# bminixhofer/zett

Measured on AMD Instinct MI355X. Metric: predicted token-embeddings/sec (full target vocab), higher is better.
Workload: dtype f16

## Files before the change

zett_amd/csrc/rowops.hip.h:

```cpp
#pragma once

#include <hip/hip_runtime.h>
#include <stdint.h>

#include <type_traits>

#include "gemm.hip.h"
#include "scan.hip.h"

namespace zett {



struct PlanArrays {
    int32_t* row_count;
    int32_t* row_offset;
    uint8_t* row_uniform;
    int32_t* id_flag;
    int32_t* id_slot;
    int32_t* id_list;
    int32_t* tok_slot;
    int32_t* tok_pos;
    int32_t* tok_row;
    int32_t* tok_pkey;
    int32_t* pair_flag;
    int32_t* pair_slot;
    int32_t* tok_pair;
    int32_t* pair_tslot;
    int32_t* pair_pos;
    uint8_t* tok_key;
    int32_t* err;
    int32_t* counters;
    int32_t n_pair_keys;
};

static __global__ void plan_rows_kernel(const int32_t* __restrict__ sfm, int64_t n_rows, int seq, int pad, int lam,
                                 int n_ids, PlanArrays p) {
    const int64_t n = (int64_t)blockIdx.x * blockDim.x + threadIdx.x;
    if (n >= n_rows) return;
    const int32_t* row = sfm + n * seq;
    int visible = 0;
    for (int j = 0; j < seq; ++j) {
        const int id = row[j];
        if (id < 0 || id >= n_ids) {
            atomicMax(p.err, (int)(n < 0x7ffffffe ? n + 1 : 0x7fffffff));
            p.row_count[n] = 0;
            p.row_uniform[n] = 2;
            return;
        }
        visible += (id != pad);
    }
    const bool uniform = (visible + lam) == 0;
    int count;
    if (uniform) {
        count = seq;
        for (int j = 0; j < seq; ++j) p.id_flag[row[j]] = 1;
    } else {
        count = visible + lam + (row[0] == pad ? 1 : 0);
        for (int j = 0; j < seq; ++j)
            if (j == 0 || row[j] != pad) p.id_flag[row[j]] = 1;
    }
    p.row_count[n] = count;
    p.row_uniform[n] = uniform ? 1 : 0;
}

static __global__ __launch_bounds__(1024) void exclusive_scan_kernel(const int32_t* __restrict__ in,
                                                              int32_t* __restrict__ out, int64_t n) {
    __shared__ int32_t s_waves[16];
    const int t = threadIdx.x;
    const int64_t per = (n + 1023) / 1024;
    const int64_t b = (int64_t)t * per, e = (b + per < n) ? b + per : n;
    int32_t s = 0;
    for (int64_t i = b; i < e; ++i) s += in[i];
    int32_t total;
    int32_t run = block_exclusive_scan<1024>(s, s_waves, &total);
    for (int64_t i = b; i < e; ++i) { const int32_t v = in[i]; out[i] = run; run += v; }
    if (t == 1023) out[n] = total;
}

constexpr int SCAN_CHUNK = 4096;

static __global__ __launch_bounds__(256) void scan_chunk_sums_kernel(const int32_t* __restrict__ in, int64_t n, int32_t* __restrict__ sums) {
    __shared__ int32_t s_waves[4];
    const int64_t base = (int64_t)blockIdx.x * SCAN_CHUNK + threadIdx.x * 16;
    int32_t s = 0;
#pragma unroll
    for (int k = 0; k < 16; ++k) { const int64_t i = base + k; if (i < n) s += in[i]; }
    int32_t total;
    block_exclusive_scan<256>(s, s_waves, &total);
    if (threadIdx.x == 0) sums[blockIdx.x] = total;
}

static __global__ __launch_bounds__(256) void scan_apply_kernel(const int32_t* __restrict__ in, int64_t n, const int32_t* __restrict__ offs,
                                                         int32_t* __restrict__ out) {
    __shared__ int32_t s_waves[4];
    const int64_t base = (int64_t)blockIdx.x * SCAN_CHUNK + threadIdx.x * 16;
    int32_t v[16];
    int32_t s = 0;
#pragma unroll
    for (int k = 0; k < 16; ++k) { const int64_t i = base + k; v[k] = i < n ? in[i] : 0; s += v[k]; }
    int32_t run = offs[blockIdx.x] + block_exclusive_scan<256>(s, s_waves);
#pragma unroll
    for (int k = 0; k < 16; ++k) { const int64_t i = base + k; if (i < n) out[i] = run; run += v[k]; }
    if (blockIdx.x == gridDim.x - 1 && threadIdx.x == 0) out[n] = offs[gridDim.x];
}

inline void launch_exclusive_scan(const int32_t* in, int32_t* out, int64_t n, int32_t* scratch, hipStream_t st) {
    if (n <= SCAN_CHUNK * 4) {
        hipLaunchKernelGGL(exclusive_scan_kernel, dim3(1), dim3(1024), 0, st, in, out, n);
        return;
    }
    const int chunks = (int)((n + SCAN_CHUNK - 1) / SCAN_CHUNK);
    int32_t* sums = scratch;
    int32_t* offs = scratch + chunks;
    hipLaunchKernelGGL(scan_chunk_sums_kernel, dim3(chunks), dim3(256), 0, st, in, n, sums);
    hipLaunchKernelGGL(exclusive_scan_kernel, dim3(1), dim3(1024), 0, st, (const int32_t*)sums, offs, (int64_t)chunks);
    hipLaunchKernelGGL(scan_apply_kernel, dim3(chunks), dim3(256), 0, st, in, n, (const int32_t*)offs, out);
}

static __global__ void plan_tokens_kernel(const int32_t* __restrict__ sfm, int64_t n_rows, int seq, int pad, int lam,
                                   int n_ids, PlanArrays p) {
    const int64_t n = (int64_t)blockIdx.x * blockDim.x + threadIdx.x;
    if (n >= n_rows) return;
    const int32_t* row = sfm + n * seq;
    int t = p.row_offset[n];
    if (p.row_uniform[n] == 2) return;
    const bool uniform = p.row_uniform[n] == 1;
    const int lp = seq + lam;
    for (int j = 0; j < seq; ++j) {
        const int id = row[j];
        const bool vis = id != pad;
        if (uniform || vis || j == 0) {
            p.tok_slot[t] = p.id_slot[id];
            p.tok_pos[t] = j;
            p.tok_row[t] = (int32_t)n;
            p.tok_key[t] = vis ? 1 : 0;
            if (p.pair_flag) { const int key = id * lp + j; p.tok_pkey[t] = key; p.pair_flag[key] = 1; }
            ++t;
        }
    }
    if (lam) {
        p.tok_slot[t] = -1;
        p.tok_pos[t] = seq;
        p.tok_row[t] = (int32_t)n;
        p.tok_key[t] = 1;
        if (p.pair_flag) { const int key = n_ids * lp + seq; p.tok_pkey[t] = key; p.pair_flag[key] = 1; }
    }
}

static __global__ void plan_pairs_kernel(int64_t n_rows, PlanArrays p) {
    const int64_t t = (int64_t)blockIdx.x * blockDim.x + threadIdx.x;
    if (t >= p.row_offset[n_rows]) return;
    const int ps = p.pair_slot[p.tok_pkey[t]];
    p.tok_pair[t] = ps;
    p.pair_tslot[ps] = p.tok_slot[t];
    p.pair_pos[ps] = p.tok_pos[t];
}

__device__ __forceinline__ int chunk_row(int t_rel, int row_rel, bool first, int rows, const int32_t* cls_slot);
static __global__ void pair_rows_kernel(int m, int tok0, int64_t row0, int rows, PlanArrays p, int32_t* __restrict__ brow_pair,
                                        const int32_t* __restrict__ cls_slot) {
    const int t = blockIdx.x * blockDim.x + threadIdx.x;
    if (t >= m) return;
    const int n = p.tok_row[tok0 + t];
    brow_pair[chunk_row(t, (int)(n - row0), p.row_offset[n] == tok0 + t, rows, cls_slot)] = p.tok_pair[tok0 + t];
}

static __global__ void plan_idlist_kernel(int n_ids, PlanArrays p) {
    const int id = blockIdx.x * blockDim.x + threadIdx.x;
    if (id < n_ids && p.id_flag[id]) p.id_list[p.id_slot[id]] = id;
    if (id == 0) {
        p.counters[0] = p.id_slot[n_ids];
        p.counters[1] = p.err[0];
        p.counters[2] = p.n_pair_keys ? p.pair_slot[p.n_pair_keys] : 0;
    }
}

__device__ __forceinline__ float wave_sum(float v) {
#pragma unroll
    for (int off = 32; off > 0; off >>= 1) v += __shfl_xor(v, off, 64);
    return v;
}

__device__ __forceinline__ float block_sum_256(float v, float* red ) {
    v = wave_sum(v);
    __syncthreads();
    if ((threadIdx.x & 63) == 0) red[threadIdx.x >> 6] = v;
    __syncthreads();
    return red[0] + red[1] + red[2] + red[3];
}

template <typename T> __device__ __forceinline__ void store_lo4(T* dst, float4 v);
template <> __device__ __forceinline__ void store_lo4<float>(float* dst, float4 v) { *(float4*)dst = v; }
template <> __device__ __forceinline__ void store_lo4<bf16_t>(bf16_t* dst, float4 v) {
    *(uint2*)dst = make_uint2(pack2_lo<bf16_t>(v.x, v.y), pack2_lo<bf16_t>(v.z, v.w));
}
template <> __device__ __forceinline__ void store_lo4<f16_t>(f16_t* dst, float4 v) {
    *(uint2*)dst = make_uint2(pack2_lo<f16_t>(v.x, v.y), pack2_lo<f16_t>(v.z, v.w));
}

template <int SRC_DTYPE> __device__ __forceinline__ float4 load_src4(const void* base, size_t elem);
template <> __device__ __forceinline__ float4 load_src4<0>(const void* base, size_t e) {
    return *(const float4*)((const float*)base + e);
}
template <> __device__ __forceinline__ float4 load_src4<1>(const void* base, size_t e) {
    const uint2 u = *(const uint2*)((const uint16_t*)base + e);
    typedef __attribute__((ext_vector_type(4))) _Float16 f16x4;
    const f16x4 hv = __builtin_bit_cast(f16x4, u);
    return make_float4((float)hv[0], (float)hv[1], (float)hv[2], (float)hv[3]);
}
template <> __device__ __forceinline__ float4 load_src4<2>(const void* base, size_t e) {
    const uint2 u = *(const uint2*)((const uint16_t*)base + e);
    return make_float4(__uint_as_float(u.x << 16), __uint_as_float(u.x & 0xffff0000u),
                       __uint_as_float(u.y << 16), __uint_as_float(u.y & 0xffff0000u));
}

template <typename T, int SRC_DTYPE>
__global__ __launch_bounds__(256) void gather_src_kernel(const int32_t* __restrict__ id_list, int slot0, int n_slots,
                                                         const void* __restrict__ src, int e_in, int v0,
                                                         const float* __restrict__ fallback,
                                                         const float* __restrict__ sc_w, const float* __restrict__ sc_b,
                                                         T* __restrict__ out, int32_t* __restrict__ range_flag) {
    const int s = blockIdx.x;
    if (s >= n_slots) return;
    const int id = id_list[slot0 + s];
    T* dst = out + (size_t)s * e_in;
    bool bad = false;
    auto chk = [&](float4 v) {
        if (LoRange<T>::checked)
            bad |= out_of_range(v.x, LoRange<T>::limit) | out_of_range(v.y, LoRange<T>::limit) | out_of_range(v.z, LoRange<T>::limit) |
                   out_of_range(v.w, LoRange<T>::limit);
    };
    if (id >= v0) {
        const float* f = fallback + (size_t)(id - v0) * e_in;
        for (int c = threadIdx.x * 4; c < e_in; c += 1024) { const float4 v = *(const float4*)(f + c); chk(v); store_lo4<T>(dst + c, v); }
    } else {
        const size_t base = (size_t)id * e_in;
        for (int c = threadIdx.x * 4; c < e_in; c += 1024) {
            float4 v = load_src4<SRC_DTYPE>(src, base + c);
            if (sc_w) {
                const float4 w = *(const float4*)(sc_w + c), b = *(const float4*)(sc_b + c);
                v.x = w.x * v.x + b.x; v.y = w.y * v.y + b.y; v.z = w.z * v.z + b.z; v.w = w.w * v.w + b.w;
            }
            chk(v);
            store_lo4<T>(dst + c, v);
        }
    }
    range_report(range_flag, bad, ZETT_RANGE_BIT_SOURCE);
}

struct LnEmbed {
    const float* table;
    const int32_t* tok_slot;
    const int32_t* tok_pos;
    const float* type0;
    const float* pos_emb;
    const float* lang;
    int lang_pos;
    const int32_t* tok_row;
    const int32_t* row_offset;
    int64_t row0;
    int rows;
    const void* table_lo;
    const float* table_stats;
    const float* table_gamma;
    const float* table_beta;
    const int32_t* cls_slot;
};

__device__ __forceinline__ int chunk_row(int t_rel, int row_rel, bool first, int rows, const int32_t* cls_slot) {
    return first ? (cls_slot ? cls_slot[row_rel] : row_rel) : rows + t_rel - row_rel - 1;
}

struct LnReadout {
    const float* bias_w;
    const float* bias_b;
    float* out_bias;
    const void* in_lo;
    const int64_t* bias_rows;
    int32_t* range_flag;
};

template <typename BT> __device__ __forceinline__ void ln_readout_store(const LnReadout& ro, int r, float v) {
    if constexpr (std::is_void<BT>::value) {
        ro.out_bias[r] = v;
    } else {
        const int64_t d = ro.bias_rows ? ro.bias_rows[r] : (int64_t)r;
        if (d < 0) return;
        ((BT*)ro.out_bias)[d] = to_lo<BT>(v);
        range_report(ro.range_flag, dest_overflow<BT>(v), ZETT_RANGE_BIT_DEST);
    }
}

constexpr int LN_MAX_VEC = 8;

template <typename T, bool EMBED, int TPR = 256, bool READOUT = false, typename BT = void>
__global__ __launch_bounds__(256) void layernorm_rows_kernel(const float* __restrict__ in, int ld_in, int rows, int H,
                                                             const float* __restrict__ gamma,
                                                             const float* __restrict__ beta, float eps,
                                                             float* __restrict__ out_f32, T* __restrict__ out_lo,
                                                             float* __restrict__ stats_out, float* __restrict__ sum_out,
                                                             LnEmbed emb, int tok0, LnReadout readout) {
    __shared__ float red[4];
    const int r = blockIdx.x * (256 / TPR) + (int)threadIdx.x / TPR;
    if (r >= rows) return;
    const int nvec = H >> 2;
    const int tid = threadIdx.x % TPR;
    auto row_sum = [&](float x_) { return TPR == 256 ? block_sum_256(x_, red) : wave_sum(x_); };
    const float* x = nullptr;
    const float* posr = nullptr;
    bool is_lang = false;
    int ro = r;
    const T* tbl_lo = nullptr;
    float2 tbl_st = make_float2(0.f, 1.f);
    if constexpr (EMBED) {
        const int slot = emb.tok_slot[tok0 + r];
        is_lang = slot < 0;
        if (emb.table_lo && !is_lang) {
            tbl_lo = (const T*)emb.table_lo + (size_t)slot * H;
            tbl_st = *(const float2*)(emb.table_stats + 2 * (size_t)slot);
            x = emb.lang;
        } else
        x = is_lang ? emb.lang : emb.table + (size_t)slot * H;
        posr = emb.pos_emb + (size_t)emb.tok_pos[tok0 + r] * H;
        if (emb.tok_row) {
            const int n = emb.tok_row[tok0 + r];
            ro = chunk_row(r, (int)(n - emb.row0), emb.row_offset[n] == tok0 + r, emb.rows, emb.cls_slot);
        }
// ... 564 lines not shown
```

zett_amd/csrc/zett_hip.hip:

```cpp
#include <hip/hip_runtime.h>

#include <algorithm>
#include <cstdlib>
#include <cmath>
#include <cstdarg>
#include <cstdio>
#include <cstring>
#include <map>
#include <string>
#include <type_traits>
#include <vector>

#include "../../include/zett_hip.h"
#include "common.hip.h"
#include "gemm.hip.h"
#include "gemm_launch.hip.h"
#include "rowops.hip.h"
#include "rowops_launch.hip.h"
#include "retok.hip.h"
#include "lexical.hip.h"
#include "partition.hip.h"

using namespace zett;

// ... 43 lines not shown
    int table_lo = 1;
    int gemm_group = 0;
    int gemm4d_min_k = 512;
    int gemm_variant = 0;
    struct PlanSlot {
        DevBuf i32, u8;
        int32_t* host = nullptr;
        size_t host_ints = 0;
        hipEvent_t done = nullptr;
        hipEvent_t released = nullptr;
        const int32_t* sfm = nullptr;
        int64_t n_rows = 0;
        int seq = 0;
        bool pair_plan = false;
        const int32_t* ext_id_slot = nullptr;
        bool pending = false;
    } plan[2];
    PlanSlot table_plan;
    struct ExtTable { const void* table = nullptr; const float* stats = nullptr; const int32_t* id_slot = nullptr; } ext;
    int plan_cur = 0;
    hipStream_t plan_stream = nullptr;
    hipEvent_t plan_fork = nullptr;
    DevBuf table, x0, yf, yt, big, pre, ctx, cf, ct, lnstats, lnparts;
    hipEvent_t out_ready[2] = {nullptr, nullptr};
    bool out_recorded = false;
    int range_accumulate = 0;
    int32_t* range_word = nullptr;
    int32_t* range_host = nullptr;
    DevBuf dest_word, dest_stage[2], dest_sink;
    int32_t* dest_host = nullptr;
    hipEvent_t dest_checked = nullptr;
    int single_rows = 1;
    int64_t single_rows_last = 0;
    DevBuf single_map;
    void* single_host = nullptr;
    size_t single_host_bytes = 0;
    hipEvent_t single_copied = nullptr;
    std::vector<hipEvent_t> ev;
    size_t ev_used = 0;
    std::vector<zett_gemm_record> gemm_log;
    zett_stats stats{};
};

namespace {

size_t elt_size(int precision) { return precision == ZETT_PREC_F32 ? 4 : 2; }

bool is_gemm_weight(const std::string& n) {
    static const char* suffixes[] = {"input_projection.0.weight", "dense1.weight", "dense2.weight",
                                     "query.weight", "key.weight", "value.weight", "dense.weight",
                                     "output_projection.1.weight", "output_projection_out.1.weight"};
    for (const char* s : suffixes) {
        const size_t ls = strlen(s);
        if (n.size() >= ls && n.compare(n.size() - ls, ls, s) == 0) return true;
    }
    return false;
}

void expected_shapes(const zett_config& c, std::map<std::string, std::vector<int64_t>>& s) {
    const int64_t H = c.hidden, I = c.intermediate;
    auto proj = [&](const std::string& p) {
        s[p + "dense1.weight"] = {I, H}; s[p + "dense1.bias"] = {I};
        s[p + "dense2.weight"] = {H, I}; s[p + "dense2.bias"] = {H};
        s[p + "ln.weight"] = {H}; s[p + "ln.bias"] = {H};
    };
    if (c.embed_lang) s["lang_embeddings.weight"] = {c.n_langs, H};
    s["model.embeddings.token_type_embeddings.weight"] = {1, H};
    s["model.embeddings.LayerNorm.weight"] = {H};
    s["model.embeddings.LayerNorm.bias"] = {H};
    s["model.embeddings.position_embeddings.weight"] = {c.max_positions, H};
    for (int l = 0; l < c.layers; ++l) {
        const std::string p = "model.encoder.layer." + std::to_string(l) + ".";
        for (const char* q : {"query", "key", "value"}) {
            s[p + "attention.self." + q + ".weight"] = {H, H};
            s[p + "attention.self." + q + ".bias"] = {H};
        }
        s[p + "attention.output.dense.weight"] = {H, H}; s[p + "attention.output.dense.bias"] = {H};
        s[p + "attention.output.LayerNorm.weight"] = {H}; s[p + "attention.output.LayerNorm.bias"] = {H};
        s[p + "intermediate.dense.weight"] = {I, H}; s[p + "intermediate.dense.bias"] = {I};
        s[p + "output.dense.weight"] = {H, I}; s[p + "output.dense.bias"] = {H};
        s[p + "output.LayerNorm.weight"] = {H}; s[p + "output.LayerNorm.bias"] = {H};
    }
    s["fallback_embeddings.weight"] = {c.n_extra, c.n_in_embd};
    s["input_projection.0.weight"] = {H, c.n_in_embd}; s["input_projection.0.bias"] = {H};
    proj("input_projection.1.");
    proj("output_projection.0.");
    const int64_t w0 = c.single_head ? c.n_in_embd : c.n_embd;
    s["output_projection.1.weight"] = {w0, H}; s["output_projection.1.bias"] = {w0};
    if (c.separate_out && !c.single_head) {
        proj("output_projection_out.0.");
        s["output_projection_out.1.weight"] = {c.n_embd, H}; s["output_projection_out.1.bias"] = {c.n_embd};
    }
    if (c.rescale) {
        s["in_scaler.w"] = {1, c.n_in_embd}; s["in_scaler.b"] = {1, c.n_in_embd};
        s["scaler.w"] = {1, c.n_embd}; s["scaler.b"] = {1, c.n_embd};
        if (c.separate_out) { s["out_scaler.w"] = {1, c.n_embd}; s["out_scaler.b"] = {1, c.n_embd}; }
    }
    if (c.predict_bias) { s["bias_projection.weight"] = {1, H}; s["bias_projection.bias"] = {1}; }
}

int validate_config(const zett_config& c, int precision) {
    if (c.n_embd <= 0 || c.hidden <= 0 || c.intermediate <= 0 || c.heads <= 0 || c.layers <= 0)
        return fail(ZETT_E_INVALID, "non-positive dimension in zett_config");
    if (c.n_in_embd != (c.separate_out ? 2 * c.n_embd : c.n_embd))
        return fail(ZETT_E_INVALID, "n_in_embd must be 2*n_embd iff separate_out");
    if (c.hidden % c.heads) return fail(ZETT_E_INVALID, "hidden %d not divisible by heads %d", c.hidden, c.heads);
    const int d = c.hidden / c.heads;
    if (d < 8 || d > 512 || (d & (d - 1))) return fail(ZETT_E_INVALID, "head_dim %d unsupported (need a power of two in [8,512])", d);
    const int kq = precision == ZETT_PREC_F32 ? 32 : 64;
    for (int k : {c.n_in_embd, c.hidden, c.intermediate})
        if (k % kq) return fail(ZETT_E_INVALID, "contraction width %d is not a multiple of %d", k, kq);
    if (c.n_embd % 4) return fail(ZETT_E_INVALID, "n_embd must be a multiple of 4");
    if (c.n_extra < 1) return fail(ZETT_E_INVALID, "n_extra must be >= 1 (reference allocates max(hn_n_extra_tokens,1))");
    if (c.pad_token_id < 0) return fail(ZETT_E_INVALID, "pad_token_id is required");
    if (c.embed_lang && c.n_langs <= 0) return fail(ZETT_E_INVALID, "hn_embed_lang_id needs n_langs");
    return 0;
}

struct WorkspaceSizes {
    int64_t chunk_tokens;
    size_t table, x0, f32_rows, lo_rows, big, stats, parts;
    size_t total() const { return table + x0 + 3 * f32_rows + 3 * lo_rows + big + stats + parts; }
};

static int64_t pair_keys(const zett_config& c, int seq) {
    return ((int64_t)c.original_vocab_size + c.n_extra + 1) * (int64_t)(seq + (c.embed_lang ? 1 : 0));
}

static int64_t chunk_token_cap(const zett_config& c, size_t es) {
    const size_t wide = (size_t)std::max(c.intermediate, 3 * c.hidden);
    const size_t per_token = (size_t)c.n_in_embd * es + 3 * (size_t)c.hidden * 4 + 3 * (size_t)c.hidden * es + wide * es + 24;
    return std::max<int64_t>(131072, (int64_t)(((size_t)12 << 30) / per_token));
}

static WorkspaceSizes workspace_sizes(const zett_config& c, size_t es, int seq, int64_t Ttot, int64_t D, int64_t cap) {
    const int lam = c.embed_lang ? 1 : 0;
    WorkspaceSizes w{};
    if (cap <= 0) cap = chunk_token_cap(c, es);
    w.chunk_tokens = std::max<int64_t>(std::min<int64_t>(cap, std::max<int64_t>(Ttot, D)), seq + lam);
    const size_t MC = (size_t)w.chunk_tokens, MCS = MC + 768;
    const size_t wide = (size_t)std::max(c.intermediate, 3 * c.hidden);
    w.table = (size_t)D * c.hidden * 4;
    w.x0 = MCS * c.n_in_embd * es;
    w.f32_rows = MCS * c.hidden * 4;
    w.lo_rows = MCS * c.hidden * es;
    w.big = MCS * wide * es;
    w.stats = 2 * MCS * 2 * sizeof(float);
    w.parts = c.hidden % 128 == 0 ? (size_t)(c.hidden / 128) * MCS * sizeof(float2) : 0;
    return w;
}

struct PlanLayout {
    PlanArrays p{};
    int32_t* scan_tmp = nullptr;
    bool pair_plan = false;
    int64_t PK = 0;
    size_t n_clear = 0;
    size_t words = 0;
};
static PlanLayout plan_layout(const zett_hypernet* h, const zett_hypernet::PlanSlot* s, int64_t N, int seq, bool worst_case = false) {
    const zett_config& c = h->cfg;
    const int lam = c.embed_lang ? 1 : 0;
    const int64_t V = (int64_t)c.original_vocab_size + c.n_extra;
    const int64_t max_tok = N * (int64_t)(seq + lam);
    PlanLayout L;
    PlanArrays& p = L.p;
    L.PK = pair_keys(c, seq);
    L.pair_plan = worst_case || (h->pair_dedupe && c.layers >= 2 && L.PK <= std::max<int64_t>(4 * max_tok, (int64_t)1 << 23) && L.PK < (int64_t)0x7fffffff);
    int32_t* const base = s ? s->i32.as<int32_t>() : nullptr;
    auto take = [&](int32_t*& array, int64_t n) { array = base ? base + L.words : nullptr; L.words += (size_t)n; };
    take(p.id_flag, V);
    if (L.pair_plan) take(p.pair_flag, L.PK);
    take(p.err, 1);
    L.n_clear = L.words;
    take(p.row_count, N); take(p.row_offset, N + 1); take(p.counters, 3);
    take(p.id_slot, V + 1); take(p.id_list, V);
    take(p.tok_slot, max_tok); take(p.tok_pos, max_tok); take(p.tok_row, max_tok);
    p.n_pair_keys = L.pair_plan ? (int32_t)L.PK : 0;
    if (L.pair_plan) {
        take(p.tok_pkey, max_tok); take(p.tok_pair, max_tok); take(p.pair_tslot, max_tok); take(p.pair_pos, max_tok);
        take(p.pair_slot, L.PK + 1);
    }
    take(L.scan_tmp, 2 * (std::max<int64_t>(std::max<int64_t>(N, V), L.PK) / SCAN_CHUNK + 2) + 1);
    if (s) {
        p.row_uniform = s->u8.as<uint8_t>();
        p.tok_key = p.row_uniform + N;
    }
    return L;
}
static size_t plan_i32_bytes(const zett_hypernet* h, int64_t N, int seq) { return plan_layout(h, nullptr, N, seq, true).words * 4; }

static int enqueue_plan(zett_hypernet* h, zett_hypernet::PlanSlot& s, const int32_t* sfm, int64_t N, int seq, hipStream_t st) {
    const zett_config& c = h->cfg;
    const int lam = c.embed_lang ? 1 : 0;
    const int V = c.original_vocab_size + c.n_extra;
    const int64_t max_tok = N * (int64_t)(seq + lam);
    if (int rc = s.i32.reserve(plan_i32_bytes(h, N, seq))) return rc;
    if (int rc = s.u8.reserve((size_t)N + (size_t)max_tok)) return rc;
    const size_t need_ints = (size_t)N + 1 + 3;
    if (s.host_ints < need_ints) {
        if (s.host) (void)hipHostFree(s.host);
        s.host = nullptr;
        HIP_TRY(hipHostMalloc((void**)&s.host, need_ints * 4, hipHostMallocDefault));
        s.host_ints = need_ints;
    }
    if (!s.done) HIP_TRY(hipEventCreateWithFlags(&s.done, hipEventDisableTiming));
    if (!s.released) HIP_TRY(hipEventCreateWithFlags(&s.released, hipEventDisableTiming));
    const PlanLayout L = plan_layout(h, &s, N, seq);
    const PlanArrays& p = L.p;
    HIP_TRY(hipMemsetAsync(s.i32.p, 0, L.n_clear * 4, st));
    const int rb = (int)((N + 255) / 256);
    hipLaunchKernelGGL(plan_rows_kernel, dim3(rb), dim3(256), 0, st, sfm, N, seq, c.pad_token_id, lam, V, p);
    launch_exclusive_scan(p.row_count, p.row_offset, N, L.scan_tmp, st);
    launch_exclusive_scan(p.id_flag, p.id_slot, (int64_t)V, L.scan_tmp, st);
    {
        PlanArrays pt = p;
        if (h->ext.id_slot) pt.id_slot = const_cast<int32_t*>(h->ext.id_slot);
        hipLaunchKernelGGL(plan_tokens_kernel, dim3(rb), dim3(256), 0, st, sfm, N, seq, c.pad_token_id, lam, V, pt);
    }
    if (L.pair_plan) {
        launch_exclusive_scan(p.pair_flag, p.pair_slot, L.PK, L.scan_tmp, st);
        hipLaunchKernelGGL(plan_pairs_kernel, dim3((unsigned)((max_tok + 255) / 256)), dim3(256), 0, st, N, p);
    }
    hipLaunchKernelGGL(plan_idlist_kernel, dim3((V + 255) / 256), dim3(256), 0, st, V, p);
    HIP_TRY(hipGetLastError());
    HIP_TRY(hipMemcpyAsync(s.host, p.row_offset, ((size_t)N + 1 + 3) * 4, hipMemcpyDeviceToHost, st));
    HIP_TRY(hipEventRecord(s.done, st));
    s.sfm = sfm; s.n_rows = N; s.seq = seq; s.pair_plan = L.pair_plan; s.ext_id_slot = h->ext.id_slot;
    return 0;
}

template <typename T>
int do_forward(zett_hypernet* h, const int32_t* sfm, int64_t N, int seq, const void* src, int src_dtype, const zett_dest* dest,
               int lang_index, float* out_in, float* out_out, float* out_bias, hipStream_t st);
template <typename T>
int do_table_rows(zett_hypernet* h, const int32_t* id_list, int first, int count, const void* src, int src_dtype, void* table_out, float* stats_out, hipStream_t st);

constexpr int CALL_EMPTY = 1;
struct CallCheck {
    int64_t n_rows = 0; int32_t seq = 1;
    bool shape = true;
    bool empty_ok = false;
    bool null_arg = false, null_first = false;
    const char* null_text = "null tensor argument";
    bool encoder = false, need_out_out = false; int32_t lang_index = 0;
    bool source = false; int src_dtype = ZETT_F32; int64_t v_src = 0;
    const char* table_mode = nullptr;
};
int check_call(const zett_hypernet* h, const CallCheck& k) {
    if (!h) return fail(ZETT_E_INVALID, "null handle");
    if (!h->finalized) return fail(ZETT_E_STATE, "zett_finalize has not been called");
    const zett_config& c = h->cfg;
    if (k.null_first && k.null_arg) return fail(ZETT_E_INVALID, "%s", k.null_text);
    if (k.shape && (k.n_rows < (k.empty_ok ? 0 : 1) || k.seq < 1)) return fail(ZETT_E_INVALID, "bad surface-form shape [%lld, %d]", (long long)k.n_rows, k.seq);
    if (k.encoder && k.seq + (c.embed_lang ? 1 : 0) > c.max_positions)
        return fail(ZETT_E_INDEX, "sequence %d exceeds position_embeddings (%d rows)", k.seq, c.max_positions);
    if (k.shape && k.n_rows == 0) return CALL_EMPTY;
    if (k.null_arg) return fail(ZETT_E_INVALID, "%s", k.null_text);
    if (k.need_out_out) return fail(ZETT_E_INVALID, "out_out is required when separate_out_embeddings is set");
    if (k.source) {
        if (!is_dtype(k.src_dtype)) return fail(ZETT_E_INVALID, "unknown source dtype %d", k.src_dtype);
        if (k.v_src < c.original_vocab_size)
            return fail(ZETT_E_INDEX, "source_embeddings has %lld rows, config.original_vocab_size is %d", (long long)k.v_src, c.original_vocab_size);
    }
    if (k.encoder && c.embed_lang && (k.lang_index < 0 || k.lang_index >= c.n_langs)) return fail(ZETT_E_INDEX, "lang_index %d outside [0,%d)", k.lang_index, c.n_langs);
    if (k.shape && k.n_rows * (int64_t)(k.seq + 1) >= (int64_t)0x7fffffff) return fail(ZETT_E_INVALID, "too many positions for one call");
    if (k.table_mode && h->precision == ZETT_PREC_F32) return fail(ZETT_E_INVALID, "%s: the folded 16-bit table exists in the 16-bit modes only", k.table_mode);
    return 0;
}

}

extern "C" {

const char* zett_last_error(void) { return g_err.c_str(); }
int zett_abi_version(void) { return ZETT_ABI_VERSION; }

int zett_create(const zett_config* cfg, int device, int precision, zett_hypernet** out) {
    if (!cfg || !out) return fail(ZETT_E_INVALID, "null argument");
    if (precision != ZETT_PREC_BF16 && precision != ZETT_PREC_F32 && precision != ZETT_PREC_F16) return fail(ZETT_E_INVALID, "unknown precision %d", precision);
    if (int rc = validate_config(*cfg, precision)) return rc;
    int ndev = 0;
    HIP_TRY(hipGetDeviceCount(&ndev));
    if (device < 0 || device >= ndev) return fail(ZETT_E_INVALID, "device %d out of range (%d visible)", device, ndev);
    ZETT_ON_DEVICE(device);
    auto* h = new zett_hypernet();
    h->cfg = *cfg;
    h->device = device;
    h->precision = precision;
    if (hipMalloc((void**)&h->range_word, 64) != hipSuccess || hipHostMalloc((void**)&h->range_host, 64, hipHostMallocDefault) != hipSuccess ||
        hipMemset(h->range_word, 0, 64) != hipSuccess) {
        if (h->range_word) (void)hipFree(h->range_word);
        if (h->range_host) (void)hipHostFree(h->range_host);
        delete h;
        return fail(ZETT_E_HIP, "allocation of the range word failed");
    }
    *out = h;
    return 0;
}

int zett_destroy(zett_hypernet* h) {
    if (!h) return 0;
    ::zett::DeviceScope _scope(h->device);
    for (auto& kv : h->w) {
        if (kv.second.f32) (void)hipFree(kv.second.f32);
        if (kv.second.lo && kv.second.lo != (void*)kv.second.f32) (void)hipFree(kv.second.lo);
    }
    for (void* p : h->owned) (void)hipFree(p);
    for (DevBuf* b : {&h->table, &h->x0, &h->yf, &h->yt, &h->big, &h->pre, &h->ctx, &h->cf, &h->ct, &h->lnstats, &h->lnparts, &h->dest_word, &h->dest_stage[0], &h->dest_stage[1], &h->dest_sink, &h->single_map})
        b->release();
    if (h->single_host) (void)hipHostFree(h->single_host);
    if (h->single_copied) (void)hipEventDestroy(h->single_copied);
    for (zett_hypernet::PlanSlot* psp : {&h->plan[0], &h->plan[1], &h->table_plan}) {
        zett_hypernet::PlanSlot& ps = *psp;
        ps.i32.release(); ps.u8.release();
        if (ps.host) (void)hipHostFree(ps.host);
        if (ps.done) (void)hipEventDestroy(ps.done);
        if (ps.released) (void)hipEventDestroy(ps.released);
    }
    if (h->plan_stream) (void)hipStreamDestroy(h->plan_stream);
    if (h->plan_fork) (void)hipEventDestroy(h->plan_fork);
    if (h->range_word) (void)hipFree(h->range_word);
    if (h->range_host) (void)hipHostFree(h->range_host);
    if (h->dest_host) (void)hipHostFree(h->dest_host);
    if (h->dest_checked) (void)hipEventDestroy(h->dest_checked);
    for (hipEvent_t e : h->out_ready) if (e) (void)hipEventDestroy(e);
    for (hipEvent_t e : h->lane_ev) if (e) (void)hipEventDestroy(e);
    if (h->lane_stream) (void)hipStreamDestroy(h->lane_stream);
    for (hipEvent_t e : h->ev) (void)hipEventDestroy(e);
    delete h;
    return 0;
}

int zett_load_weight(zett_hypernet* h, const char* name, const void* data, int dtype, const int64_t* shape, int ndim) {
    if (!h || !name || !data || !shape || ndim < 1) return fail(ZETT_E_INVALID, "null argument");
    if (h->finalized) return fail(ZETT_E_STATE, "weights are frozen after zett_finalize");
    std::map<std::string, std::vector<int64_t>> exp;
    expected_shapes(h->cfg, exp);
    const std::string n(name);
    auto it = exp.find(n);
    if (it == exp.end()) return 0;
    std::vector<int64_t> got(shape, shape + ndim);
    if (got != it->second) {
        std::string a, b;
        for (auto v : got) a += std::to_string(v) + ",";
        for (auto v : it->second) b += std::to_string(v) + ",";
        return fail(ZETT_E_INVALID, "%s: shape [%s] does not match the config's [%s]", name, a.c_str(), b.c_str());
    }
    ZETT_ON_DEVICE(h->device);
    size_t numel = 1;
    for (auto v : got) numel *= (size_t)v;
    Tensor& t = h->w[n];
    if (t.f32) { (void)hipFree(t.f32); t.f32 = nullptr; }
    t.shape = got;
    t.numel = numel;
    HIP_TRY(hipMalloc((void**)&t.f32, numel * 4));
    if (dtype == ZETT_F32) {
        HIP_TRY(hipMemcpy(t.f32, data, numel * 4, hipMemcpyDefault));
    } else if (dtype == ZETT_F16 || dtype == ZETT_BF16) {
        void* stage = nullptr;
        HIP_TRY(hipMalloc(&stage, numel * 2));
        hipError_t e = hipMemcpy(stage, data, numel * 2, hipMemcpyDefault);
        if (e == hipSuccess) {
            const int blocks = (int)std::min<size_t>((numel + 255) / 256, 65535);
            if (dtype == ZETT_F16) hipLaunchKernelGGL(convert_to_f32_kernel<1>, dim3(blocks), dim3(256), 0, 0, stage, t.f32, numel);
            else hipLaunchKernelGGL(convert_to_f32_kernel<2>, dim3(blocks), dim3(256), 0, 0, stage, t.f32, numel);
            e = hipDeviceSynchronize();
        }
        (void)hipFree(stage);
        if (e != hipSuccess) return fail(ZETT_E_HIP, "upload of %s failed: %s", name, hipGetErrorString(e));
    } else {
        return fail(ZETT_E_INVALID, "unknown dtype %d", dtype);
    }
    return 0;
}

int zett_finalize(zett_hypernet* h) {
// ... 1166 lines not shown
```

Measured before the change: 627,100.

## Batch plan scans into one segmented launch and fuse token/pair/idlist kernels

Pair-key flags are now set in plan_rows_kernel, so all three exclusive scans (row counts, id flags, pair flags) can run as one segmented scan of at most three launches. The separate token, pair and id-list kernels are merged into a single tail kernel. Chunk sums are stored in place in the output arrays instead of a scratch buffer. The aim is to cut kernel launch count and serialization in the planning phase, at the cost of more complex segment indexing and a strided chunk-sum scan.

```diff
diff --git a/zett_amd/csrc/rowops.hip.h b/zett_amd/csrc/rowops.hip.h
--- a/zett_amd/csrc/rowops.hip.h
+++ b/zett_amd/csrc/rowops.hip.h
@@ -51,110 +51,159 @@
         visible += (id != pad);
     }
     const bool uniform = (visible + lam) == 0;
-    int count;
-    if (uniform) {
-        count = seq;
-        for (int j = 0; j < seq; ++j) p.id_flag[row[j]] = 1;
-    } else {
-        count = visible + lam + (row[0] == pad ? 1 : 0);
-        for (int j = 0; j < seq; ++j)
-            if (j == 0 || row[j] != pad) p.id_flag[row[j]] = 1;
-    }
+    const int count = uniform ? seq : visible + lam + (row[0] == pad ? 1 : 0);
+    const int lp = seq + lam;
+    for (int j = 0; j < seq; ++j) {
+        const int id = row[j];
+        if (uniform || j == 0 || id != pad) {
+            p.id_flag[id] = 1;
+            if (p.pair_flag) p.pair_flag[id * lp + j] = 1;
+        }
+    }
+    if (lam && p.pair_flag) p.pair_flag[n_ids * lp + seq] = 1;
     p.row_count[n] = count;
     p.row_uniform[n] = uniform ? 1 : 0;
 }
 
-static __global__ __launch_bounds__(1024) void exclusive_scan_kernel(const int32_t* __restrict__ in,
-                                                              int32_t* __restrict__ out, int64_t n) {
-    __shared__ int32_t s_waves[16];
+__device__ __forceinline__ void workgroup_exclusive_scan(const int32_t* in, int32_t* out, int64_t n, int64_t stride, int32_t* total_out,
+                                                         int32_t* s_waves ) {
     const int t = threadIdx.x;
     const int64_t per = (n + 1023) / 1024;
     const int64_t b = (int64_t)t * per, e = (b + per < n) ? b + per : n;
     int32_t s = 0;
-    for (int64_t i = b; i < e; ++i) s += in[i];
+    for (int64_t i = b; i < e; ++i) s += in[i * stride];
     int32_t total;
     int32_t run = block_exclusive_scan<1024>(s, s_waves, &total);
-    for (int64_t i = b; i < e; ++i) { const int32_t v = in[i]; out[i] = run; run += v; }
-    if (t == 1023) out[n] = total;
+    for (int64_t i = b; i < e; ++i) { const int32_t v = in[i * stride]; out[i * stride] = run; run += v; }
+    if (t == 1023) *total_out = total;
+}
+
+static __global__ __launch_bounds__(1024) void exclusive_scan_kernel(const int32_t* __restrict__ in,
+                                                              int32_t* __restrict__ out, int64_t n) {
+    __shared__ int32_t s_waves[16];
+    workgroup_exclusive_scan(in, out, n, 1, out + n, s_waves);
+}
+
+constexpr int SCAN_MAX_SEGMENTS = 3;
+struct ScanSegments {
+    const int32_t* in[SCAN_MAX_SEGMENTS];
+    int32_t* out[SCAN_MAX_SEGMENTS];
+    int64_t n[SCAN_MAX_SEGMENTS];
+    int32_t chunk0[SCAN_MAX_SEGMENTS + 1];
+    int32_t count;
+};
+__device__ __forceinline__ int scan_segment_of(const ScanSegments& g, int chunk) {
+    int s = 0;
+#pragma unroll
+    for (int k = 1; k < SCAN_MAX_SEGMENTS; ++k) s += (k < g.count && chunk >= g.chunk0[k]) ? 1 : 0;
+    return s;
+}
+__device__ __forceinline__ int scan_segment_chunk0(const ScanSegments& g, int s) {
+    int v = g.chunk0[0];
+#pragma unroll
+    for (int k = 1; k <= SCAN_MAX_SEGMENTS; ++k) v = s == k ? g.chunk0[k] : v;
+    return v;
+}
+template <typename A> __device__ __forceinline__ A scan_pick(const A (&a)[SCAN_MAX_SEGMENTS], int s) {
+    A v = a[0];
+#pragma unroll
+    for (int k = 1; k < SCAN_MAX_SEGMENTS; ++k) v = s == k ? a[k] : v;
+    return v;
 }
 
 constexpr int SCAN_CHUNK = 4096;
-
-static __global__ __launch_bounds__(256) void scan_chunk_sums_kernel(const int32_t* __restrict__ in, int64_t n, int32_t* __restrict__ sums) {
+__host__ __device__ inline int64_t scan_chunks(int64_t n) { return n > SCAN_CHUNK ? (n + SCAN_CHUNK - 1) / SCAN_CHUNK : 1; }
+
+static __global__ __launch_bounds__(1024) void exclusive_scan_segments_kernel(ScanSegments g, int chunk_sums) {
+    __shared__ int32_t s_waves[16];
+#pragma unroll
+    for (int s = 0; s < SCAN_MAX_SEGMENTS; ++s) {
+        if (s >= g.count) continue;
+        if (chunk_sums) workgroup_exclusive_scan(g.out[s], g.out[s], scan_chunks(g.n[s]), SCAN_CHUNK, g.out[s] + g.n[s], s_waves);
+        else workgroup_exclusive_scan(g.in[s], g.out[s], g.n[s], 1, g.out[s] + g.n[s], s_waves);
+    }
+}
+
+static __global__ __launch_bounds__(256) void scan_chunk_sums_kernel(ScanSegments g) {
     __shared__ int32_t s_waves[4];
-    const int64_t base = (int64_t)blockIdx.x * SCAN_CHUNK + threadIdx.x * 16;
+    const int seg = scan_segment_of(g, blockIdx.x);
+    const int32_t* __restrict__ in = scan_pick(g.in, seg);
+    const int64_t n = scan_pick(g.n, seg);
+    const int64_t chunk = (int64_t)(blockIdx.x - scan_segment_chunk0(g, seg)) * SCAN_CHUNK, base = chunk + threadIdx.x * 16;
     int32_t s = 0;
 #pragma unroll
     for (int k = 0; k < 16; ++k) { const int64_t i = base + k; if (i < n) s += in[i]; }
     int32_t total;
     block_exclusive_scan<256>(s, s_waves, &total);
-    if (threadIdx.x == 0) sums[blockIdx.x] = total;
-}
-
-static __global__ __launch_bounds__(256) void scan_apply_kernel(const int32_t* __restrict__ in, int64_t n, const int32_t* __restrict__ offs,
-                                                         int32_t* __restrict__ out) {
+    if (threadIdx.x == 0) scan_pick(g.out, seg)[chunk] = total;
+}
+
+static __global__ __launch_bounds__(256) void scan_apply_kernel(ScanSegments g) {
     __shared__ int32_t s_waves[4];
-    const int64_t base = (int64_t)blockIdx.x * SCAN_CHUNK + threadIdx.x * 16;
+    const int seg = scan_segment_of(g, blockIdx.x);
+    const int32_t* __restrict__ in = scan_pick(g.in, seg);
+    int32_t* out = scan_pick(g.out, seg);
+    const int64_t n = scan_pick(g.n, seg);
+    const int64_t chunk = (int64_t)(blockIdx.x - scan_segment_chunk0(g, seg)) * SCAN_CHUNK, base = chunk + threadIdx.x * 16;
+    const int32_t offset = out[chunk];
     int32_t v[16];
     int32_t s = 0;
 #pragma unroll
     for (int k = 0; k < 16; ++k) { const int64_t i = base + k; v[k] = i < n ? in[i] : 0; s += v[k]; }
-    int32_t run = offs[blockIdx.x] + block_exclusive_scan<256>(s, s_waves);
+    int32_t run = offset + block_exclusive_scan<256>(s, s_waves);
 #pragma unroll
     for (int k = 0; k < 16; ++k) { const int64_t i = base + k; if (i < n) out[i] = run; run += v[k]; }
-    if (blockIdx.x == gridDim.x - 1 && threadIdx.x == 0) out[n] = offs[gridDim.x];
-}
-
-inline void launch_exclusive_scan(const int32_t* in, int32_t* out, int64_t n, int32_t* scratch, hipStream_t st) {
-    if (n <= SCAN_CHUNK * 4) {
-        hipLaunchKernelGGL(exclusive_scan_kernel, dim3(1), dim3(1024), 0, st, in, out, n);
+}
+
+inline void launch_exclusive_scans(ScanSegments g, hipStream_t st) {
+    int64_t total = 0;
+    for (int s = 0; s < g.count; ++s) total += g.n[s];
+    if (total <= SCAN_CHUNK * 4) {
+        hipLaunchKernelGGL(exclusive_scan_segments_kernel, dim3(1), dim3(1024), 0, st, g, 0);
         return;
     }
-    const int chunks = (int)((n + SCAN_CHUNK - 1) / SCAN_CHUNK);
-    int32_t* sums = scratch;
-    int32_t* offs = scratch + chunks;
-    hipLaunchKernelGGL(scan_chunk_sums_kernel, dim3(chunks), dim3(256), 0, st, in, n, sums);
-    hipLaunchKernelGGL(exclusive_scan_kernel, dim3(1), dim3(1024), 0, st, (const int32_t*)sums, offs, (int64_t)chunks);
-    hipLaunchKernelGGL(scan_apply_kernel, dim3(chunks), dim3(256), 0, st, in, n, (const int32_t*)offs, out);
-}
-
-static __global__ void plan_tokens_kernel(const int32_t* __restrict__ sfm, int64_t n_rows, int seq, int pad, int lam,
-                                   int n_ids, PlanArrays p) {
+    int chunks = 0;
+    for (int s = 0; s < g.count; ++s) { g.chunk0[s] = chunks; chunks += (int)scan_chunks(g.n[s]); }
+    for (int s = g.count; s <= SCAN_MAX_SEGMENTS; ++s) g.chunk0[s] = chunks;
+    hipLaunchKernelGGL(scan_chunk_sums_kernel, dim3(chunks), dim3(256), 0, st, g);
+    hipLaunchKernelGGL(exclusive_scan_segments_kernel, dim3(1), dim3(1024), 0, st, g, 1);
+    hipLaunchKernelGGL(scan_apply_kernel, dim3(chunks), dim3(256), 0, st, g);
+}
+
+static __global__ void plan_tail_kernel(const int32_t* __restrict__ sfm, int64_t n_rows, int seq, int pad, int lam,
+                                        int n_ids, PlanArrays p, const int32_t* __restrict__ tok_id_slot) {
     const int64_t n = (int64_t)blockIdx.x * blockDim.x + threadIdx.x;
-    if (n >= n_rows) return;
+    if (n < n_ids && p.id_flag[n]) p.id_list[p.id_slot[n]] = (int32_t)n;
+    if (n == 0) {
+        p.counters[0] = p.id_slot[n_ids];
+        p.counters[1] = p.err[0];
+        p.counters[2] = p.n_pair_keys ? p.pair_slot[p.n_pair_keys] : 0;
+    }
+    if (n >= n_rows || p.row_uniform[n] == 2) return;
     const int32_t* row = sfm + n * seq;
     int t = p.row_offset[n];
-    if (p.row_uniform[n] == 2) return;
     const bool uniform = p.row_uniform[n] == 1;
     const int lp = seq + lam;
+    auto position = [&](int slot, int pos, bool vis, int key) {
+        p.tok_slot[t] = slot;
+        p.tok_pos[t] = pos;
+        p.tok_row[t] = (int32_t)n;
+        p.tok_key[t] = vis ? 1 : 0;
+        if (p.pair_flag) {
+            const int ps = p.pair_slot[key];
+            p.tok_pkey[t] = key;
+            p.tok_pair[t] = ps;
+            p.pair_tslot[ps] = slot;
+            p.pair_pos[ps] = pos;
+        }
+        ++t;
+    };
     for (int j = 0; j < seq; ++j) {
         const int id = row[j];
         const bool vis = id != pad;
-        if (uniform || vis || j == 0) {
-            p.tok_slot[t] = p.id_slot[id];
-            p.tok_pos[t] = j;
-            p.tok_row[t] = (int32_t)n;
-            p.tok_key[t] = vis ? 1 : 0;
-            if (p.pair_flag) { const int key = id * lp + j; p.tok_pkey[t] = key; p.pair_flag[key] = 1; }
-            ++t;
-        }
-    }
-    if (lam) {
-        p.tok_slot[t] = -1;
-        p.tok_pos[t] = seq;
-        p.tok_row[t] = (int32_t)n;
-        p.tok_key[t] = 1;
-        if (p.pair_flag) { const int key = n_ids * lp + seq; p.tok_pkey[t] = key; p.pair_flag[key] = 1; }
-    }
-}
-
-static __global__ void plan_pairs_kernel(int64_t n_rows, PlanArrays p) {
-    const int64_t t = (int64_t)blockIdx.x * blockDim.x + threadIdx.x;
-    if (t >= p.row_offset[n_rows]) return;
-    const int ps = p.pair_slot[p.tok_pkey[t]];
-    p.tok_pair[t] = ps;
-    p.pair_tslot[ps] = p.tok_slot[t];
-    p.pair_pos[ps] = p.tok_pos[t];
+        if (uniform || vis || j == 0) position(tok_id_slot[id], j, vis, id * lp + j);
+    }
+    if (lam) position(-1, seq, true, n_ids * lp + seq);
 }
 
 __device__ __forceinline__ int chunk_row(int t_rel, int row_rel, bool first, int rows, const int32_t* cls_slot);
@@ -164,16 +213,6 @@
     if (t >= m) return;
     const int n = p.tok_row[tok0 + t];
     brow_pair[chunk_row(t, (int)(n - row0), p.row_offset[n] == tok0 + t, rows, cls_slot)] = p.tok_pair[tok0 + t];
-}
-
-static __global__ void plan_idlist_kernel(int n_ids, PlanArrays p) {
-    const int id = blockIdx.x * blockDim.x + threadIdx.x;
-    if (id < n_ids && p.id_flag[id]) p.id_list[p.id_slot[id]] = id;
-    if (id == 0) {
-        p.counters[0] = p.id_slot[n_ids];
-        p.counters[1] = p.err[0];
-        p.counters[2] = p.n_pair_keys ? p.pair_slot[p.n_pair_keys] : 0;
-    }
 }
 
 __device__ __forceinline__ float wave_sum(float v) {
diff --git a/zett_amd/csrc/zett_hip.hip b/zett_amd/csrc/zett_hip.hip
--- a/zett_amd/csrc/zett_hip.hip
+++ b/zett_amd/csrc/zett_hip.hip
@@ -219,7 +219,6 @@
 
 struct PlanLayout {
     PlanArrays p{};
-    int32_t* scan_tmp = nullptr;
     bool pair_plan = false;
     int64_t PK = 0;
     size_t n_clear = 0;
@@ -248,7 +247,7 @@
         take(p.tok_pkey, max_tok); take(p.tok_pair, max_tok); take(p.pair_tslot, max_tok); take(p.pair_pos, max_tok);
         take(p.pair_slot, L.PK + 1);
     }
-    take(L.scan_tmp, 2 * (std::max<int64_t>(std::max<int64_t>(N, V), L.PK) / SCAN_CHUNK + 2) + 1);
+    L.words += (size_t)(2 * (std::max<int64_t>(std::max<int64_t>(N, V), L.PK) / SCAN_CHUNK + 2) + 1);
     if (s) {
         p.row_uniform = s->u8.as<uint8_t>();
         p.tok_key = p.row_uniform + N;
@@ -278,18 +277,15 @@
     HIP_TRY(hipMemsetAsync(s.i32.p, 0, L.n_clear * 4, st));
     const int rb = (int)((N + 255) / 256);
     hipLaunchKernelGGL(plan_rows_kernel, dim3(rb), dim3(256), 0, st, sfm, N, seq, c.pad_token_id, lam, V, p);
-    launch_exclusive_scan(p.row_count, p.row_offset, N, L.scan_tmp, st);
-    launch_exclusive_scan(p.id_flag, p.id_slot, (int64_t)V, L.scan_tmp, st);
-    {
-        PlanArrays pt = p;
-        if (h->ext.id_slot) pt.id_slot = const_cast<int32_t*>(h->ext.id_slot);
-        hipLaunchKernelGGL(plan_tokens_kernel, dim3(rb), dim3(256), 0, st, sfm, N, seq, c.pad_token_id, lam, V, pt);
-    }
-    if (L.pair_plan) {
-        launch_exclusive_scan(p.pair_flag, p.pair_slot, L.PK, L.scan_tmp, st);
-        hipLaunchKernelGGL(plan_pairs_kernel, dim3((unsigned)((max_tok + 255) / 256)), dim3(256), 0, st, N, p);
-    }
-    hipLaunchKernelGGL(plan_idlist_kernel, dim3((V + 255) / 256), dim3(256), 0, st, V, p);
+    ScanSegments scans{};
+    scans.in[0] = p.row_count; scans.out[0] = p.row_offset; scans.n[0] = N;
+    scans.in[1] = p.id_flag; scans.out[1] = p.id_slot; scans.n[1] = V;
+    scans.count = 2;
+    if (L.pair_plan) { scans.in[2] = p.pair_flag; scans.out[2] = p.pair_slot; scans.n[2] = L.PK; scans.count = 3; }
+    launch_exclusive_scans(scans, st);
+    const int32_t* tok_id_slot = h->ext.id_slot ? h->ext.id_slot : p.id_slot;
+    const int64_t tail = std::max<int64_t>(N, V);
+    hipLaunchKernelGGL(plan_tail_kernel, dim3((unsigned)((tail + 255) / 256)), dim3(256), 0, st, sfm, N, seq, c.pad_token_id, lam, V, p, tok_id_slot);
     HIP_TRY(hipGetLastError());
     HIP_TRY(hipMemcpyAsync(s.host, p.row_offset, ((size_t)N + 1 + 3) * 4, hipMemcpyDeviceToHost, st));
     HIP_TRY(hipEventRecord(s.done, st));
```

New measurement: 627,000. About the same (-0.0%).
